# lasgroup/Model-based-policy-optimizers

Measured on AMD Instinct MI355X. Metric: model-rollout transitions/sec + SAC updates/sec, Pendulum 5-ens h=5, higher is better.
Workload: dtype f32

## Files before the change

### include/mbpo_hip.h

```cpp
#ifndef MBPO_HIP_H
#define MBPO_HIP_H

#include <stdint.h>

#ifdef __cplusplus
extern "C" {
#endif

#define MBPO_OK 0
#define MBPO_ERR_ARG (-1)
#define MBPO_ERR_UNSUPPORTED (-2)
#define MBPO_ERR_LAUNCH (-3)

#define MBPO_MAX_LAYERS 8

#define MBPO_ACT_SWISH 0
#define MBPO_ACT_RELU 1
#define MBPO_ACT_TANH 2

typedef struct mbpo_mlp_desc {
  const float *params;
  int64_t net_stride;
  int32_t n_nets;
  int32_t n_layers;
// ... 77 lines not shown
  int32_t ppo_extras, env_major;
  int32_t step_index, n_steps;
  const float *action;
  const float *raw_action;
  const float *log_prob;
  const float *reward;
  const float *x_next;
  const float *sys_done;
  const float *first_obs;
  float *obs, *steps, *done;
  float *transitions;
  int32_t row_len;
} mbpo_episode_step_desc;

int mbpo_episode_step(const mbpo_episode_step_desc *d, void *stream);

int mbpo_replay_insert(float *data, int64_t max_size, int32_t row_len, int32_t *state, const float *rows,
                       int64_t n_rows, void *stream);
int mbpo_replay_gather(const float *data, int64_t max_size, int32_t row_len, const int32_t *state, const int32_t *idx,
                       int64_t n, float *out, void *stream);
int mbpo_replay_sample(const float *data, int64_t max_size, int32_t row_len, const int32_t *state, uint64_t seed,
                       uint64_t offset, const uint64_t *rng_dev, int64_t n, int32_t *idx_out, float *out, void *stream);

int mbpo_philox_permutation(uint64_t seed, uint64_t offset, const uint64_t *rng_dev, int64_t n, int32_t *perm,
                            uint32_t *workspace, void *stream);

int64_t mbpo_running_stats_workspace_floats(int32_t x_dim);
int mbpo_running_stats_reduce(const float *rows, int64_t n_rows, int32_t row_len, int32_t col_off, int32_t x_dim,
                              const float *stats, float *sums, float *workspace, int32_t pass, void *stream);
int mbpo_running_stats_apply(float *stats, const float *sums, int32_t x_dim, float std_min, float std_max, void *stream);
int mbpo_running_stats_update(const float *rows, int64_t n_rows, int32_t row_len, int32_t col_off, int32_t x_dim, float *stats,
                              float *sums, float *workspace, float std_min, float std_max, void *stream);

int mbpo_gae_scan(const float *truncation, const float *termination, const float *rewards, const float *values,
                  const float *bootstrap, float *vs, float *advantages, int64_t B, int32_t T, float gamma,
                  float lam, int32_t time_major, void *stream);
int mbpo_lambda_return_scan(const float *rewards, const float *next_values, float *returns, int64_t B, int32_t T,
                            float gamma, float lam, int32_t time_major, void *stream);
int mbpo_gae_scan_discounts(const float *truncation, const float *termination, const float *rewards, const float *values,
                            const float *bootstrap, const float *discounts, float *vs, float *advantages, int64_t B,
                            int32_t T, float lam, int32_t time_major, void *stream);

typedef struct mbpo_sac_desc {
  int32_t x_dim, u_dim;
  int32_t policy_layers;
  int32_t policy_dims[MBPO_MAX_LAYERS + 1];
  int32_t q_layers;
  int32_t q_dims[MBPO_MAX_LAYERS + 1];
  int32_t policy_activation, q_activation;
  float *params, *target_q, *adam_m, *adam_v, *step_count, *grads;
  float *workspace;
  float *metrics;
  float *metrics_accum;
  const float *batch;
  int32_t batch_size, row_len;
  const float *norm_mean, *norm_std;
  const float *noise_alpha, *noise_critic, *noise_actor;
  uint64_t seed, offset;
  const uint64_t *rng_dev;
  float discounting, reward_scaling, target_entropy, tau;
  float lr_policy, lr_q, lr_alpha, wd_policy, wd_q, wd_alpha, max_grad_norm;
  float grad_scale;
  int32_t non_equidistant_time;
  float continuous_discounting, min_time_between_switches, max_time_between_switches, env_dt;
} mbpo_sac_desc;

// ... 157 lines not shown
```

### model-based-policy-optimizers_amd/csrc/replay.hip

```cpp
#include "common.hpp"
#include <stdlib.h>

struct ReplayPos {
  int pos, roll, head;
};

__device__ __forceinline__ ReplayPos replay_plan(const int *state, long long max_size, long long n) {
  ReplayPos p;
  long long pos = state[0];
  long long roll = max_size - pos - n;
  if (roll > 0) roll = 0;
  p.roll = (int)roll;
  p.pos = (int)(pos + roll);
  p.head = (int)(((long long)state[2] - roll) % max_size);
  return p;
}

__global__ void __launch_bounds__(256) k_replay_insert(float *data, long long max_size, int D, const int *state,
                                                        const float *rows, long long n_rows) {
  const ReplayPos p = replay_plan(state, max_size, n_rows);
  const long long s0 = ((long long)p.pos + p.head) % max_size;
  const long long n1 = (max_size - s0) < n_rows ? (max_size - s0) : n_rows;
  const long long e1 = n1 * D, total = n_rows * D;
  float *dst1 = data + s0 * D;
  const long long gtid = (long long)blockIdx.x * blockDim.x + threadIdx.x, gsz = (long long)gridDim.x * blockDim.x;
  const bool vec = ((e1 | total) & 3) == 0 && ((((unsigned long long)dst1) | ((unsigned long long)data) | ((unsigned long long)rows)) & 15ull) == 0;
  if (vec) {
    const f32x4 *src = reinterpret_cast<const f32x4 *>(rows);
    f32x4 *d1 = reinterpret_cast<f32x4 *>(dst1), *d2 = reinterpret_cast<f32x4 *>(data);
    const long long q1 = e1 >> 2, qt = total >> 2;
    for (long long i = gtid; i < qt; i += gsz) {
      const f32x4 v = src[i];
      if (i < q1) d1[i] = v;
      else d2[i - q1] = v;
    }
  } else {
    for (long long i = gtid; i < total; i += gsz) {
      const float v = rows[i];
      if (i < e1) dst1[i] = v;
      else data[i - e1] = v;
    }
  }
}

__global__ void k_replay_advance(int *state, long long max_size, long long n_rows) {
  if (threadIdx.x == 0 && blockIdx.x == 0) {
    const ReplayPos p = replay_plan(state, max_size, n_rows);
    long long newpos = ((long long)p.pos + n_rows) % (max_size + 1);
    long long sp = (long long)state[1] + p.roll;
    state[0] = (int)newpos;
    state[1] = (int)(sp > 0 ? sp : 0);
    state[2] = p.head;
    state[3] = (int)((unsigned)state[3] + (unsigned)n_rows);
  }
}

extern "C" int mbpo_replay_insert(float *data, int64_t max_size, int32_t row_len, int32_t *state, const float *rows,
                                  int64_t n_rows, void *stream) {
  MBPO_REQUIRE(data && state, MBPO_ERR_ARG, "replay_insert: null pointer");
  MBPO_REQUIRE(max_size > 0 && max_size < (1LL << 31) - 1 && row_len > 0, MBPO_ERR_ARG, "replay_insert: bad max_size/row_len");
  MBPO_REQUIRE(n_rows >= 0 && n_rows <= max_size, MBPO_ERR_ARG,
               "replay_insert: %lld rows do not fit a buffer of %lld rows", (long long)n_rows, (long long)max_size);
  if (n_rows == 0) return MBPO_OK;
  MBPO_REQUIRE(rows, MBPO_ERR_ARG, "replay_insert: null rows");
  long long total = n_rows * row_len;
  int grid = (int)((total + 255) / 256 < 2048 ? (total + 255) / 256 : 2048);
  hipStream_t st = (hipStream_t)stream;
  hipLaunchKernelGGL(k_replay_insert, dim3(grid), dim3(256), 0, st, data, (long long)max_size, row_len, state, rows,
                     (long long)n_rows);
  hipLaunchKernelGGL(k_replay_advance, dim3(1), dim3(64), 0, st, state, (long long)max_size, (long long)n_rows);
  MBPO_CHECK_LAUNCH("replay_insert");
  return MBPO_OK;
}

static int gather_rows_per_block(int row_len) {
  const int pieces = (row_len & 3) == 0 ? row_len >> 2 : row_len;
  int rb = (2048 + pieces - 1) / pieces;
  return rb < 1 ? 1 : (rb > 256 ? 256 : rb);
}

template <bool SAMPLE>
__global__ void __launch_bounds__(256) k_replay_gather(const float *data, long long max_size, int D, const int *state,
                                                        const int *idx, unsigned long long seed, unsigned long long offset,
                                                        const unsigned long long *rng_dev, long long n, int *idx_out, float *out, int RB) {
  __shared__ long long s_phys[256];
  if (SAMPLE) {
    const RngKey rk = rng_resolve(seed, offset, rng_dev);
    seed = rk.seed;
    offset = rk.offset;
  }
  const int head = state[2];
  const int lo = state[1], hi = state[0];
  const int tid = threadIdx.x;
  const bool vec = (D & 3) == 0 && ((((unsigned long long)data) | ((unsigned long long)out)) & 15ull) == 0;
  for (long long row0 = (long long)blockIdx.x * RB; row0 < n; row0 += (long long)gridDim.x * RB) {
    const long long j = row0 + tid;
    if (tid < RB && j < n) {
      long long li;
      if (SAMPLE) {
        li = philox_randint(seed, offset, MBPO_STREAM_REPLAY, (unsigned long long)j, lo, hi);
        if (idx_out) idx_out[j] = (int)li;
      } else {
        li = idx[j];
      }
      long long w = li % max_size;
      if (w < 0) w += max_size;
      s_phys[tid] = (w + head) % max_size;
    }
    __syncthreads();
    const int rows_here = (int)((n - row0) < RB ? (n - row0) : RB);
    if (vec) {
      const int D4 = D >> 2, total = rows_here * D4;
      const f32x4 *src = reinterpret_cast<const f32x4 *>(data);
      f32x4 *dst = reinterpret_cast<f32x4 *>(out) + row0 * D4;
      for (int e = tid; e < total; e += 256) {
        const int r = e / D4, c = e - r * D4;
        dst[e] = src[s_phys[r] * D4 + c];
      }
    } else {
      const int total = rows_here * D;
      float *dst = out + row0 * D;
      for (int e = tid; e < total; e += 256) {
        const int r = e / D, c = e - r * D;
        dst[e] = data[s_phys[r] * D + c];
      }
    }
    __syncthreads();
  }
}

extern "C" int mbpo_replay_gather(const float *data, int64_t max_size, int32_t row_len, const int32_t *state,
                                  const int32_t *idx, int64_t n, float *out, void *stream) {
  MBPO_REQUIRE(data && state, MBPO_ERR_ARG, "replay_gather: null pointer");
  MBPO_REQUIRE(max_size > 0 && row_len > 0 && n >= 0, MBPO_ERR_ARG, "replay_gather: bad sizes");
  if (n == 0) return MBPO_OK;
  MBPO_REQUIRE(idx && out, MBPO_ERR_ARG, "replay_gather: null idx/out");
  const int RB = gather_rows_per_block(row_len);
  int grid = (int)((n + RB - 1) / RB < 4096 ? (n + RB - 1) / RB : 4096);
  hipLaunchKernelGGL(k_replay_gather<false>, dim3(grid), dim3(256), 0, (hipStream_t)stream, data, (long long)max_size, row_len,
                     state, idx, 0ull, 0ull, (const unsigned long long *)nullptr, (long long)n, (int *)nullptr, out, RB);
  MBPO_CHECK_LAUNCH("replay_gather");
  return MBPO_OK;
}

extern "C" int mbpo_replay_sample(const float *data, int64_t max_size, int32_t row_len, const int32_t *state, uint64_t seed,
                                  uint64_t offset, const uint64_t *rng_dev, int64_t n, int32_t *idx_out, float *out,
                                  void *stream) {
  MBPO_REQUIRE(data && state, MBPO_ERR_ARG, "replay_sample: null pointer");
  MBPO_REQUIRE(max_size > 0 && row_len > 0 && n >= 0, MBPO_ERR_ARG, "replay_sample: bad sizes");
  if (n == 0) return MBPO_OK;
  MBPO_REQUIRE(out, MBPO_ERR_ARG, "replay_sample: null out");
  const int RB = gather_rows_per_block(row_len);
  int grid = (int)((n + RB - 1) / RB < 4096 ? (n + RB - 1) / RB : 4096);
  hipLaunchKernelGGL(k_replay_gather<true>, dim3(grid), dim3(256), 0, (hipStream_t)stream, data, (long long)max_size, row_len,
                     state, (const int *)nullptr, (unsigned long long)seed, (unsigned long long)offset, (const unsigned long long *)rng_dev, (long long)n, idx_out, out, RB);
  MBPO_CHECK_LAUNCH("replay_sample");
  return MBPO_OK;
}

#define STATS_WGS 512

__device__ __forceinline__ float wave_sum(float v) {
#pragma unroll
  for (int o = 32; o > 0; o >>= 1) v += __shfl_down(v, o, 64);
  return v;
}

template <int PASS>
__global__ void __launch_bounds__(256) k_stats_partial(const float *rows, long long n_rows, int D, int col_off, int X,
                                                        const float *stats, const float *sums, float *partial) {
  const int tid = threadIdx.x;
  const float *mean = stats + 1;
  const int rows_per_pass = 256 / X;
  const int c = tid % X, r0 = tid / X;
  float acc = 0.f;
  if (r0 < rows_per_pass) {
    const float m = mean[c];
    float upd = 0.f;
    if (PASS == 1) upd = sums[1 + c] / (stats[0] + sums[0]);
    for (long long r = (long long)blockIdx.x * rows_per_pass + r0; r < n_rows; r += (long long)gridDim.x * rows_per_pass) {
      float d = rows[r * D + col_off + c] - m;
      acc += (PASS == 0) ? d : d * (d - upd);
    }
  }
  __shared__ float s_all[256];
  s_all[tid] = acc;
  __syncthreads();
  if (tid < X) {
    float a = 0.f;
    for (int t = tid; t < rows_per_pass * X; t += X) a += s_all[t];
    partial[(long long)blockIdx.x * X + tid] = a;
  }
}

__device__ __forceinline__ float stats_column_sums(const float *partial, int n_parts, int X, float *s_sl) {
  const int tid = threadIdx.x;
  const int nsl = 256 / X, c = tid % X, sl = tid / X;
  float acc = 0.f;
  if (sl < nsl) {
    int g = sl;
    for (; g + 7 * nsl < n_parts; g += 8 * nsl) {
      float v[8];
#pragma unroll
      for (int k = 0; k < 8; ++k) v[k] = partial[(long long)(g + k * nsl) * X + c];
#pragma unroll
      for (int k = 0; k < 8; ++k) acc += v[k];
    }
    for (; g < n_parts; g += nsl) acc += partial[(long long)g * X + c];
  }
  s_sl[tid] = acc;
  __syncthreads();
  float a = 0.f;
  if (tid < X)
    for (int k = 0; k < nsl; ++k) a += s_sl[k * X + tid];
  __syncthreads();
  return a;
}

template <int PASS>
__global__ void __launch_bounds__(256) k_stats_sums(const float *partial, int n_parts, int X, long long n_rows, float *sums) {
  __shared__ float s_sl[256];
  const int tid = threadIdx.x;
  const float a = stats_column_sums(partial, n_parts, X, s_sl);
  if (tid < X) sums[1 + PASS * X + tid] = a;
  if (PASS == 0 && tid == 0) sums[0] = (float)n_rows;
// ... 21 lines not shown
    hipLaunchKernelGGL(k_stats_sums<0>, dim3(1), dim3(256), 0, st, workspace, grid, x_dim, (long long)n_rows, sums);
  } else {
    hipLaunchKernelGGL(k_stats_partial<1>, dim3(grid), dim3(256), 0, st, rows, (long long)n_rows, row_len, col_off, x_dim, stats,
                       (const float *)sums, workspace);
    hipLaunchKernelGGL(k_stats_sums<1>, dim3(1), dim3(256), 0, st, workspace, grid, x_dim, (long long)n_rows, sums);
  }
  MBPO_CHECK_LAUNCH("running_stats_reduce");
  return MBPO_OK;
}

__global__ void k_stats_apply(float *stats, const float *sums, int X, float std_min, float std_max) {
  const int c = threadIdx.x;
  const float count = stats[0] + sums[0];
  if (c < X && count > 0.f) {
    float *mean = stats + 1, *sv = stats + 1 + X, *sd = stats + 1 + 2 * X;
    mean[c] = mean[c] + sums[1 + c] / count;
    float nsv = sv[c] + sums[1 + X + c];
    sv[c] = nsv;
    float s = sqrtf(fmaxf(nsv, 0.f) / count);
    sd[c] = fminf(fmaxf(s, std_min), std_max);
  }
  __syncthreads();
  if (c == 0) stats[0] = count;
}

extern "C" int mbpo_running_stats_apply(float *stats, const float *sums, int32_t x_dim, float std_min, float std_max, void *stream) {
  MBPO_REQUIRE(stats && sums, MBPO_ERR_ARG, "running_stats_apply: null pointer");
  MBPO_REQUIRE(x_dim > 0 && x_dim <= 128, MBPO_ERR_ARG, "running_stats_apply: x_dim out of range");
  hipLaunchKernelGGL(k_stats_apply, dim3(1), dim3(128), 0, (hipStream_t)stream, stats, sums, x_dim, std_min, std_max);
  MBPO_CHECK_LAUNCH("running_stats_apply");
  return MBPO_OK;
}

__global__ void __launch_bounds__(256) k_stats_pass1_fused(const float *rows, long long n_rows, int D, int col_off, int X,
                                                           const float *stats, const float *partial0, int n_parts0, float *sums,
                                                           float *partial1) {
  __shared__ float s_all[256];
  __shared__ float s_sum0[128];
  const int tid = threadIdx.x;
  const float tot = stats_column_sums(partial0, n_parts0, X, s_all);
  if (tid < X) {
    s_sum0[tid] = tot;
    if (blockIdx.x == 0) sums[1 + tid] = tot;
  }
  if (blockIdx.x == 0 && tid == 0) sums[0] = (float)n_rows;
  __syncthreads();
  const float *mean = stats + 1;
  const int rows_per_pass = 256 / X;
  const int c = tid % X, r0 = tid / X;
  float acc = 0.f;
  if (r0 < rows_per_pass) {
    const float m = mean[c];
    const float upd = s_sum0[c] / (stats[0] + (float)n_rows);
    for (long long r = (long long)blockIdx.x * rows_per_pass + r0; r < n_rows; r += (long long)gridDim.x * rows_per_pass) {
      float d = rows[r * D + col_off + c] - m;
      acc += d * (d - upd);
    }
  }
  s_all[tid] = acc;
  __syncthreads();
  if (tid < X) {
    float a = 0.f;
    for (int t = tid; t < rows_per_pass * X; t += X) a += s_all[t];
    partial1[(long long)blockIdx.x * X + tid] = a;
  }
}

__global__ void __launch_bounds__(256) k_stats_sums1_apply(const float *partial1, int n_parts, int X, float *sums, float *stats,
                                                           float std_min, float std_max) {
  __shared__ float s_sl[256];
  const int c = threadIdx.x;
  const float a = stats_column_sums(partial1, n_parts, X, s_sl);
  const float count = stats[0] + sums[0];
  if (c < X) {
    sums[1 + X + c] = a;
    if (count > 0.f) {
      float *mean = stats + 1, *sv = stats + 1 + X, *sd = stats + 1 + 2 * X;
      mean[c] = mean[c] + sums[1 + c] / count;
      float nsv = sv[c] + a;
      sv[c] = nsv;
      float s = sqrtf(fmaxf(nsv, 0.f) / count);
      sd[c] = fminf(fmaxf(s, std_min), std_max);
    }
  }
  __syncthreads();
  if (c == 0) stats[0] = count;
}

extern "C" int mbpo_running_stats_update(const float *rows, int64_t n_rows, int32_t row_len, int32_t col_off, int32_t x_dim,
                                         float *stats, float *sums, float *workspace, float std_min, float std_max, void *stream) {
  MBPO_REQUIRE(stats && sums && workspace, MBPO_ERR_ARG, "running_stats_update: null pointer");
  MBPO_REQUIRE(x_dim > 0 && x_dim <= 128 && row_len > 0 && col_off >= 0 && col_off + x_dim <= row_len, MBPO_ERR_ARG,
               "running_stats_update: bad column range (x_dim must be <= 128)");
  MBPO_REQUIRE(n_rows >= 0 && (n_rows == 0 || rows), MBPO_ERR_ARG, "running_stats_update: bad rows");
  hipStream_t st = (hipStream_t)stream;
  int rows_per_pass = 256 / x_dim;
  long long want = (n_rows + rows_per_pass - 1) / rows_per_pass;
  int grid = (int)(want < 1 ? 1 : (want < STATS_WGS ? want : STATS_WGS));
  float *partial1 = workspace + (long long)STATS_WGS * x_dim;
  hipLaunchKernelGGL(k_stats_partial<0>, dim3(grid), dim3(256), 0, st, rows, (long long)n_rows, row_len, col_off, x_dim,
                     (const float *)stats, (const float *)sums, workspace);
  hipLaunchKernelGGL(k_stats_pass1_fused, dim3(grid), dim3(256), 0, st, rows, (long long)n_rows, row_len, col_off, x_dim,
                     (const float *)stats, (const float *)workspace, grid, sums, partial1);
  hipLaunchKernelGGL(k_stats_sums1_apply, dim3(1), dim3(256), 0, st, (const float *)partial1, grid, x_dim, sums, stats, std_min, std_max);
  MBPO_CHECK_LAUNCH("running_stats_update");
  return MBPO_OK;
}

__global__ void __launch_bounds__(256) k_perm_keys(unsigned long long seed, unsigned long long offset, const unsigned long long *rng_dev,
                                                    long long n, unsigned int *keys) {
  const RngKey rk = rng_resolve(seed, offset, rng_dev);
  const long long i = (long long)blockIdx.x * 256 + threadIdx.x;
  if (i >= n) return;
  Philox4 p = philox4x32_10((uint32_t)i, (uint32_t)((unsigned long long)i >> 32), MBPO_STREAM_PERM ^ (uint32_t)(rk.offset >> 32) * 0x9E3779B9u,
                            (uint32_t)rk.offset, (uint32_t)rk.seed, (uint32_t)(rk.seed >> 32));
  keys[i] = p.v[0];
}

__global__ void __launch_bounds__(256) k_perm_rank(const unsigned int *keys, long long n, int *perm) {
  __shared__ unsigned int s_k[1024];
  const long long i = (long long)blockIdx.x * 256 + threadIdx.x;
  const unsigned int ki = i < n ? keys[i] : 0u;
  int rank = 0;
  for (long long j0 = 0; j0 < n; j0 += 1024) {
    __syncthreads();
    for (int t = threadIdx.x; t < 1024; t += 256) s_k[t] = (j0 + t < n) ? keys[j0 + t] : 0xFFFFFFFFu;
    __syncthreads();
    const int m = (int)((n - j0) < 1024 ? (n - j0) : 1024);
    for (int t = 0; t < m; ++t) {
      const unsigned int kj = s_k[t];
      rank += (kj < ki || (kj == ki && j0 + t < i)) ? 1 : 0;
    }
  }
  if (i < n) perm[rank] = (int)i;
}

__global__ void __launch_bounds__(1024) k_perm_sort_lds(unsigned long long seed, unsigned long long offset, const unsigned long long *rng_dev,
                                                         int n, int np, int *perm, unsigned int *flag) {
// ... 123 lines not shown
```

### model-based-policy-optimizers_amd/mbpo/_hip.py

```python
from __future__ import annotations

import ctypes as C
import os
from pathlib import Path
from typing import Optional, Sequence

import torch

MBPO_MAX_LAYERS = 8
ACT_IDS = {"swish": 0, "silu": 0, "relu": 1, "tanh": 2}

SYS_PENDULUM, SYS_ENSEMBLE = 0, 1
SYS_GENERIC = 100
ENS_MEAN, ENS_TS1, ENS_TSINF = 0, 1, 2
STREAM_POLICY_NOISE, STREAM_MODEL_NOISE, STREAM_MEMBER = 1, 2, 3
REWARD_PENDULUM, REWARD_QUADRATIC, REWARD_LEARNED = 0, 1, 2

_LIB_PATH = Path(__file__).resolve().parent / "_lib" / "libmbpo_hip.so"


class P2pDesc(C.Structure):
    _fields_ = [("world", C.c_int32), ("rank", C.c_int32), ("n_max", C.c_int64), ("regions", C.c_void_p * 16)]


# ... 138 lines not shown


def load() -> C.CDLL:
    global _lib
    if _lib is not None:
        return _lib
    p = lib_path()
    if not p.exists():
        raise MbpoHipError(
            f"{p} not found: build it with `python model-based-policy-optimizers_amd/build.py` "
            "(needs hipcc; this framework has no CPU fallback)")
    lib = C.CDLL(str(p))
    lib.mbpo_version.restype = C.c_int
    lib.mbpo_last_error.restype = C.c_char_p
    lib.mbpo_ensemble_mlp_forward.restype = C.c_int
    lib.mbpo_ensemble_mlp_forward.argtypes = [C.POINTER(MlpDesc), C.c_void_p, C.c_int32, C.c_void_p, C.c_int64,
                                              C.c_void_p]
    lib.mbpo_model_rollout.restype = C.c_int
    lib.mbpo_model_rollout.argtypes = [C.POINTER(RolloutDesc), C.c_void_p]
    _bind_optional(lib)
    _lib = lib
    return lib


def _bind_optional(lib: C.CDLL) -> None:
    i32, i64, u64, f32, vp = C.c_int32, C.c_int64, C.c_uint64, C.c_float, C.c_void_p
    sigs = {
        "mbpo_replay_insert": [vp, i64, i32, vp, vp, i64, vp],
        "mbpo_replay_gather": [vp, i64, i32, vp, vp, i64, vp, vp],
        "mbpo_replay_sample": [vp, i64, i32, vp, u64, u64, vp, i64, vp, vp, vp],
        "mbpo_running_stats_reduce": [vp, i64, i32, i32, i32, vp, vp, vp, i32, vp],
        "mbpo_running_stats_apply": [vp, vp, i32, f32, f32, vp],
        "mbpo_running_stats_update": [vp, i64, i32, i32, i32, vp, vp, vp, f32, f32, vp],
        "mbpo_gae_scan": [vp, vp, vp, vp, vp, vp, vp, i64, i32, f32, f32, i32, vp],
        "mbpo_gae_scan_discounts": [vp, vp, vp, vp, vp, vp, vp, vp, i64, i32, f32, i32, vp],
        "mbpo_lambda_return_scan": [vp, vp, vp, i64, i32, f32, f32, i32, vp],
        "mbpo_critic_grads": [vp, i32, i32, vp, i32, vp, i32, vp, vp, i64, vp, vp, vp, vp, vp, vp],
        "mbpo_adamw_step": [vp, vp, vp, vp, vp, i64, f32, f32, f32, i32, vp, f32, vp, vp, vp],
        "mbpo_rng_advance": [vp, u64, vp],
        "mbpo_soft_update": [vp, vp, vp, i64, f32, vp],
        "mbpo_philox_permutation": [u64, u64, vp, i64, vp, vp, vp],
    }
    for name, argtypes in sigs.items():
        fn = getattr(lib, name, None)
        if fn is not None:
            fn.restype = C.c_int
            fn.argtypes = argtypes
    for name in ("mbpo_sac_grads", "mbpo_sac_grad_norms", "mbpo_sac_apply", "mbpo_sac_step", "mbpo_sac_finalize"):
        fn = getattr(lib, name, None)
        if fn is not None:
            fn.restype = C.c_int
            fn.argtypes = [C.POINTER(SacDesc), vp]
    fn = getattr(lib, "mbpo_sac_finalize_advance", None)
    if fn is not None:
        fn.restype = C.c_int
        fn.argtypes = [C.POINTER(SacDesc), vp, u64, vp]
    for name in ("mbpo_ppo_grads", "mbpo_ppo_apply", "mbpo_ppo_step"):
        fn = getattr(lib, name, None)
        if fn is not None:
            fn.restype = C.c_int
            fn.argtypes = [C.POINTER(PpoDesc), vp]
    fn = getattr(lib, "mbpo_ppo_workspace_floats", None)
    if fn is not None:
        fn.restype = C.c_int64
        fn.argtypes = [C.POINTER(PpoDesc)]
    fn = getattr(lib, "mbpo_critic_workspace_floats", None)
# ... 122 lines not shown
```

### model-based-policy-optimizers_amd/mbpo/ops.py

```python
from __future__ import annotations

import ctypes as C
import os
from dataclasses import dataclass
from typing import Optional, Sequence

import torch

from . import _hip
from ._hip import check, current_stream_ptr, load, mlp_desc, ptr, require_device_tensor as _req


@dataclass
class MlpSpec:
    dims: Sequence[int]
    activation: str = "swish"
    n_nets: int = 1

    @property
    def n_params(self) -> int:
        d = list(self.dims)
        return sum(d[i] * d[i + 1] + d[i + 1] for i in range(len(d) - 1))

    @property
# ... 467 lines not shown
                         std_min: float = 1e-6, std_max: float = 1e6) -> None:
    if all_reduce is None:
        lib = load()
        _req(rows, "rows"); _req(stats, "stats")
        if rows.dim() != 2 or stats.numel() != 1 + 3 * x_dim:
            raise ValueError("rows must be [n, row_len] and stats [1 + 3*x_dim]")
        if sums is None:
            sums = torch.zeros(1 + 2 * x_dim, device=rows.device, dtype=torch.float32)
        if workspace is None:
            workspace = torch.empty(stats_workspace_floats(x_dim), device=rows.device, dtype=torch.float32)
        _req(sums, "sums"); _req(workspace, "workspace")
        if workspace.numel() < stats_workspace_floats(x_dim):
            raise ValueError(f"workspace must hold {stats_workspace_floats(x_dim)} floats, got {workspace.numel()}")
        check(lib.mbpo_running_stats_update(rows.data_ptr(), rows.shape[0], rows.shape[1], col_off, x_dim, stats.data_ptr(),
                                            sums.data_ptr(), workspace.data_ptr(), std_min, std_max, current_stream_ptr()),
              "mbpo_running_stats_update")
        return
    sums = running_stats_reduce(rows, col_off, x_dim, stats, 0, sums=sums, workspace=workspace)
    if all_reduce is not None:
        all_reduce(sums)
    running_stats_reduce(rows, col_off, x_dim, stats, 1, sums=sums, workspace=workspace)
    if all_reduce is not None:
        all_reduce(sums[1 + x_dim:])
    running_stats_apply(stats, sums, x_dim, std_min, std_max)


def running_stats_apply(stats: torch.Tensor, sums: torch.Tensor, x_dim: int, std_min: float = 1e-6, std_max: float = 1e6) -> None:
    lib = load()
    _req(stats, "stats"); _req(sums, "sums")
    check(lib.mbpo_running_stats_apply(stats.data_ptr(), sums.data_ptr(), x_dim, std_min, std_max, current_stream_ptr()),
          "mbpo_running_stats_apply")


def gae_scan(truncation, termination, rewards, values, bootstrap, gamma, lam: float, time_major: bool = False):
    lib = load()
    for t, nm in ((truncation, "truncation"), (termination, "termination"), (rewards, "rewards"), (values, "values"),
                  (bootstrap, "bootstrap")):
        _req(t, nm)
    B, T = (values.shape[1], values.shape[0]) if time_major else (values.shape[0], values.shape[1])
    if bootstrap.shape != (B,):
        raise ValueError("bootstrap must be [B]")
    vs = torch.empty_like(values)
    adv = torch.empty_like(values)
    if isinstance(gamma, torch.Tensor):
        _req(gamma, "gamma")
        if gamma.shape != values.shape:
            raise ValueError("a per-element discount must have the shape of rewards/values")
        check(lib.mbpo_gae_scan_discounts(truncation.data_ptr(), termination.data_ptr(), rewards.data_ptr(), values.data_ptr(),
                                          bootstrap.data_ptr(), gamma.data_ptr(), vs.data_ptr(), adv.data_ptr(), B, T, lam,
                                          int(time_major), current_stream_ptr()), "mbpo_gae_scan_discounts")
        return vs, adv
    check(lib.mbpo_gae_scan(truncation.data_ptr(), termination.data_ptr(), rewards.data_ptr(), values.data_ptr(),
                            bootstrap.data_ptr(), vs.data_ptr(), adv.data_ptr(), B, T, gamma, lam, int(time_major),
                            current_stream_ptr()), "mbpo_gae_scan")
    return vs, adv


def lambda_return_scan(rewards, next_values, gamma: float, lam: float, time_major: bool = False):
    lib = load()
    _req(rewards, "rewards"); _req(next_values, "next_values")
    B, T = (rewards.shape[1], rewards.shape[0]) if time_major else (rewards.shape[0], rewards.shape[1])
    out = torch.empty_like(rewards)
    check(lib.mbpo_lambda_return_scan(rewards.data_ptr(), next_values.data_ptr(), out.data_ptr(), B, T, gamma, lam,
                                      int(time_major), current_stream_ptr()), "mbpo_lambda_return_scan")
    return out

# ... 573 lines not shown
```

### model-based-policy-optimizers_amd/mbpo/optimizers/policy_optimizers/sac/sac.py

```python
from __future__ import annotations

import dataclasses
import math
import os
import time
from dataclasses import dataclass
from typing import Any, Callable, Dict, List, Optional, Sequence, Tuple

import torch

from mbpo import _hip, ops
from mbpo.optimizers.policy_optimizers.brax_utils.base import State
from mbpo.parallel import DataParallel
from mbpo.replay import ReplayBufferState, UniformSamplingQueue
from mbpo.systems.brax_wrapper import BraxWrapper
from mbpo.systems.ensemble_system import lecun_uniform_flat
from mbpo.types import Transition
from mbpo.utils import keys as K

Metrics = Dict[str, Any]

SITE_ROLLOUT, SITE_SAMPLE, SITE_SGD = 1, 2, 16


# ... 195 lines not shown

        return policy

    def _norm(self, normalizer_params: RunningStatisticsState):
        if not self.normalize_observations:
            return None, None
        return normalizer_params.mean.contiguous(), normalizer_params.std.contiguous()

    def init_training_state(self, key: int) -> TrainingState:
        key_policy, key_q = K.split(key)
        gp = torch.Generator().manual_seed(key_policy % (2 ** 63))
        gq = torch.Generator().manual_seed(key_q % (2 ** 63))
        pol = ops.embed_mlp_params(lecun_uniform_flat(self.policy_dims_logical, gp), self.policy_dims_logical, self.kernel_width)
        q = torch.cat([ops.embed_mlp_params(lecun_uniform_flat(self.q_dims_logical, gq), self.q_dims_logical, self.q_width)
                       for _ in range(2)])
        params = torch.cat([pol, q, torch.tensor([self.init_log_alpha], dtype=torch.float32)]).to(self.device)
        self.dp.broadcast(params, src=0)
        self.updater.load_state(params)
        self._stats_vec.zero_()
        self._stats_vec[1 + 2 * self.x_dim:] = 1.0
        return self._training_state(env_steps=0)

    def _training_state(self, env_steps: int) -> TrainingState:
        u = self.updater
        return TrainingState(policy_optimizer_state=(u.adam_m[:u.P], u.adam_v[:u.P]), policy_params=u.policy_params,
                             q_optimizer_state=(u.adam_m[u.P:u.P + 2 * u.Q], u.adam_v[u.P:u.P + 2 * u.Q]),
                             q_params=u.q_params, target_q_params=u.target_q, gradient_steps=u.step_count,
                             env_steps=env_steps, alpha_optimizer_state=(u.adam_m[-1:], u.adam_v[-1:]),
                             alpha_params=u.log_alpha, normalizer_params=RunningStatisticsState(self._stats_vec, self.x_dim))

    def rekey(self, key: int) -> None:
        ops.set_rng(self._rng, K.PRNGKey(key), 0)

    def get_experience(self, normalizer_params: RunningStatisticsState, policy_params: torch.Tensor, env_state: State,
                       buffer_state: ReplayBufferState, key: Optional[int] = None):
        if key is not None:
            self.rekey(key)
        nm, ns = self._norm(normalizer_params)
        spec = self.env.system.rollout_spec(env_state.system_params, self.device)
        sp_out: list = []
        rows = ops.model_rollout(policy_params=policy_params, policy_spec=self.policy_spec, x_dim=self.x_dim, u_dim=self.u_dim,
                                 obs=env_state.obs, first_obs=env_state.info['first_obs'], steps=env_state.info['steps'],
                                 done=env_state.done, n_steps=self.num_env_steps_between_updates,
                                 episode_length=self.episode_length, action_repeat=self.action_repeat, norm_mean=nm,
                                 norm_std=ns, seed=0, offset=SITE_ROLLOUT << 32, rng_dev=self._rng,
                                 out=self._rollout_rows, system_params_out=sp_out, **spec)
        if sp_out:
            env_state = env_state.replace(system_params=sp_out[-1])
        ops.running_stats_update(rows, 0, self.x_dim, normalizer_params.vec, all_reduce=self._all_reduce,
                                 sums=self._stats_sums, workspace=self._stats_ws)
        buffer_state = self.replay_buffer.insert_rows(buffer_state, rows)
        return normalizer_params, env_state, buffer_state

    def sgd_step(self, transitions_rows: torch.Tensor, normalizer_params: RunningStatisticsState, key: Optional[int] = None,
                 g: int = 0, defer_clip_check: bool = False) -> None:
        if key is not None:
            self.rekey(key)
        nm, ns = self._norm(normalizer_params)
        self.updater.sgd_step(transitions_rows, nm, ns, seed=0, offset=(SITE_SGD + g) << 32, rng_dev=self._rng,
                              defer_clip_check=defer_clip_check)

    def training_step(self, training_state: TrainingState, env_state: State, buffer_state: ReplayBufferState,
                      key: Optional[int] = None):
        if key is not None:
            self.rekey(key)
        normalizer_params, env_state, buffer_state = self.get_experience(
            training_state.normalizer_params, training_state.policy_params, env_state, buffer_state)
        training_state = training_state.replace(
            env_steps=training_state.env_steps + self.env_steps_per_actor_step * self.num_env_steps_between_updates)
        buffer_state, rows = self.replay_buffer.sample_rows(buffer_state, out=self._batch_rows, seed=0,
                                                            offset=SITE_SAMPLE << 32, rng_dev=self._rng)
        B = self.batch_size
        for g in range(self.grad_updates_per_step):
            self.sgd_step(rows[g * B:(g + 1) * B], normalizer_params, g=g, defer_clip_check=True)
        self.updater.finalize(rng_dev=self._rng)
        return training_state, env_state, buffer_state

    def prefill_replay_buffer(self, training_state: TrainingState, env_state: State, buffer_state: ReplayBufferState, key: int):
        key, new_key = K.split(key)
        self.rekey(key)
        for _ in range(self.num_prefill_actor_steps):
            _, env_state, buffer_state = self.get_experience(training_state.normalizer_params, training_state.policy_params,
                                                             env_state, buffer_state)
            ops.rng_advance(self._rng)
            training_state = training_state.replace(env_steps=training_state.env_steps + self.env_steps_per_actor_step)
        return training_state, env_state, buffer_state, new_key

    def training_epoch(self, training_state: TrainingState, env_state: State, buffer_state: ReplayBufferState, key: int):
        self.updater.metrics_accum.zero_()
        n = self.num_training_steps_per_epoch
        env_steps_per = self.env_steps_per_actor_step * self.num_env_steps_between_updates
        done_steps = 0
        self.rekey(key)
        if self.use_graph and self._capturable():
            gkey, refs = self._graph_signature(training_state, env_state, buffer_state)
            if self._graph is None or self._graph_key != gkey:
                training_state, env_state, buffer_state = self.training_step(training_state, env_state, buffer_state)
                done_steps = 1
                gkey, refs = self._graph_signature(training_state, env_state, buffer_state)
                torch.cuda.synchronize()
                graph = torch.cuda.CUDAGraph()
                with torch.cuda.graph(graph):
                    self.training_step(training_state, env_state, buffer_state)
                self._graph, self._graph_key, self._graph_refs = graph, gkey, refs
# ... 171 lines not shown
```

### model-based-policy-optimizers_amd/mbpo/replay.py

```python
from __future__ import annotations

import dataclasses
from dataclasses import dataclass
from typing import Optional, Tuple

import torch

from . import ops
from .types import Transition, flatten, row_layout, unflatten
from .utils import keys as K


@dataclass
class ReplayBufferState:
    data: torch.Tensor
    state: torch.Tensor
    key: int
    insert_position: int = 0
    sample_position: int = 0
    head: int = 0
    sample_count: int = 0

    def replace(self, **kw):
        return dataclasses.replace(self, **kw)
# ... 14 lines not shown
            d.observation.device if d.observation.is_cuda else torch.device("cuda", torch.cuda.current_device()))

    def init(self, key: int) -> ReplayBufferState:
        data = torch.zeros(self.max_replay_size, self.row_len, device=self.device, dtype=torch.float32)
        state = torch.zeros(4, device=self.device, dtype=torch.int32)
        return ReplayBufferState(data=data, state=state, key=K.PRNGKey(key))

    def insert(self, buffer_state: ReplayBufferState, samples) -> ReplayBufferState:
        rows = samples if isinstance(samples, torch.Tensor) else flatten(samples)
        return self.insert_rows(buffer_state, rows)

    def sample(self, buffer_state: ReplayBufferState) -> Tuple[ReplayBufferState, Transition]:
        st, rows = self.sample_rows(buffer_state)
        return st, unflatten(rows, self.x_dim, self.u_dim, self.has_truncation, self.ppo_extras)

    def size(self, buffer_state: ReplayBufferState) -> int:
        return buffer_state.insert_position - buffer_state.sample_position

    def insert_rows(self, bs: ReplayBufferState, rows: torch.Tensor) -> ReplayBufferState:
        n = rows.shape[0]
        if n > self.max_replay_size:
            raise ValueError(f"cannot insert {n} rows into a buffer of {self.max_replay_size}")
        ops.replay_insert(bs.data, bs.state, rows.to(self.device).contiguous())
        return self.insert_mirror(bs, n)

    def insert_mirror(self, bs: ReplayBufferState, n: int) -> ReplayBufferState:
        mx = self.max_replay_size
        roll = min(0, mx - bs.insert_position - n)
        pos = bs.insert_position + roll
        return bs.replace(insert_position=(pos + n) % (mx + 1), sample_position=max(0, bs.sample_position + roll),
                          head=(bs.head - roll) % mx)

    def sample_rows(self, bs: ReplayBufferState, n: Optional[int] = None, out: Optional[torch.Tensor] = None,
                    rng_dev: Optional[torch.Tensor] = None, seed: Optional[int] = None, offset: int = 0
                    ) -> Tuple[ReplayBufferState, torch.Tensor]:
        n = self.sample_batch_size if n is None else n
        if self.size(bs) <= 0:
            raise ValueError("cannot sample from an empty replay buffer")
        key, sample_key = K.split(bs.key)
        rows = ops.replay_sample(bs.data, bs.state, n, seed=sample_key if seed is None else seed, offset=offset, out=out,
                                 rng_dev=rng_dev)
        return bs.replace(key=key, sample_count=bs.sample_count + 1), rows

    def logical_data(self, bs: ReplayBufferState) -> torch.Tensor:
        idx = (torch.arange(self.max_replay_size, device=bs.data.device) + bs.head) % self.max_replay_size
        return bs.data[idx]
```

Baseline: 18.82 million.

## Fuse replay insert/advance and sampling into the running-stats kernels

```diff
diff --git a/include/mbpo_hip.h b/include/mbpo_hip.h
--- a/include/mbpo_hip.h
+++ b/include/mbpo_hip.h
@@ -133,6 +133,13 @@
 int mbpo_running_stats_update(const float *rows, int64_t n_rows, int32_t row_len, int32_t col_off, int32_t x_dim, float *stats,
                               float *sums, float *workspace, float std_min, float std_max, void *stream);
 
+int mbpo_stats_insert(const float *rows, int64_t n_rows, int32_t row_len, int32_t col_off, int32_t x_dim, float *stats, float *sums,
+                      float *workspace, float std_min, float std_max, float *data, int64_t max_size, int32_t *state,
+                      int32_t defer_apply, void *stream);
+int mbpo_sample_stats_apply(const float *data, int64_t max_size, int32_t row_len, const int32_t *state, uint64_t seed, uint64_t offset,
+                            const uint64_t *rng_dev, int64_t n, int32_t *idx_out, float *out, int64_t n_rows_stats, int32_t x_dim,
+                            float *stats, float *sums, const float *workspace, float std_min, float std_max, void *stream);
+
 int mbpo_gae_scan(const float *truncation, const float *termination, const float *rewards, const float *values,
                   const float *bootstrap, float *vs, float *advantages, int64_t B, int32_t T, float gamma,
                   float lam, int32_t time_major, void *stream);
diff --git a/model-based-policy-optimizers_amd/csrc/replay.hip b/model-based-policy-optimizers_amd/csrc/replay.hip
--- a/model-based-policy-optimizers_amd/csrc/replay.hip
+++ b/model-based-policy-optimizers_amd/csrc/replay.hip
@@ -16,8 +16,8 @@
   return p;
 }
 
-__global__ void __launch_bounds__(256) k_replay_insert(float *data, long long max_size, int D, const int *state,
-                                                        const float *rows, long long n_rows) {
+__device__ __forceinline__ void replay_insert_copy(float *data, long long max_size, int D, const int *state, const float *rows,
+                                                   long long n_rows) {
   const ReplayPos p = replay_plan(state, max_size, n_rows);
   const long long s0 = ((long long)p.pos + p.head) % max_size;
   const long long n1 = (max_size - s0) < n_rows ? (max_size - s0) : n_rows;
@@ -43,16 +43,23 @@
   }
 }
 
+__global__ void __launch_bounds__(256) k_replay_insert(float *data, long long max_size, int D, const int *state,
+                                                        const float *rows, long long n_rows) {
+  replay_insert_copy(data, max_size, D, state, rows, n_rows);
+}
+
+__device__ __forceinline__ void replay_advance_state(int *state, long long max_size, long long n_rows) {
+  const ReplayPos p = replay_plan(state, max_size, n_rows);
+  long long newpos = ((long long)p.pos + n_rows) % (max_size + 1);
+  long long sp = (long long)state[1] + p.roll;
+  state[0] = (int)newpos;
+  state[1] = (int)(sp > 0 ? sp : 0);
+  state[2] = p.head;
+  state[3] = (int)((unsigned)state[3] + (unsigned)n_rows);
+}
+
 __global__ void k_replay_advance(int *state, long long max_size, long long n_rows) {
-  if (threadIdx.x == 0 && blockIdx.x == 0) {
-    const ReplayPos p = replay_plan(state, max_size, n_rows);
-    long long newpos = ((long long)p.pos + n_rows) % (max_size + 1);
-    long long sp = (long long)state[1] + p.roll;
-    state[0] = (int)newpos;
-    state[1] = (int)(sp > 0 ? sp : 0);
-    state[2] = p.head;
-    state[3] = (int)((unsigned)state[3] + (unsigned)n_rows);
-  }
+  if (threadIdx.x == 0 && blockIdx.x == 0) replay_advance_state(state, max_size, n_rows);
 }
 
 extern "C" int mbpo_replay_insert(float *data, int64_t max_size, int32_t row_len, int32_t *state, const float *rows,
@@ -80,10 +87,9 @@
 }
 
 template <bool SAMPLE>
-__global__ void __launch_bounds__(256) k_replay_gather(const float *data, long long max_size, int D, const int *state,
-                                                        const int *idx, unsigned long long seed, unsigned long long offset,
-                                                        const unsigned long long *rng_dev, long long n, int *idx_out, float *out, int RB) {
-  __shared__ long long s_phys[256];
+__device__ __forceinline__ void replay_gather_rows(const float *data, long long max_size, int D, const int *state, const int *idx,
+                                                   unsigned long long seed, unsigned long long offset, const unsigned long long *rng_dev,
+                                                   long long n, int *idx_out, float *out, int RB, long long *s_phys, int bid, int nblk) {
   if (SAMPLE) {
     const RngKey rk = rng_resolve(seed, offset, rng_dev);
     seed = rk.seed;
@@ -93,7 +99,7 @@
   const int lo = state[1], hi = state[0];
   const int tid = threadIdx.x;
   const bool vec = (D & 3) == 0 && ((((unsigned long long)data) | ((unsigned long long)out)) & 15ull) == 0;
-  for (long long row0 = (long long)blockIdx.x * RB; row0 < n; row0 += (long long)gridDim.x * RB) {
+  for (long long row0 = (long long)bid * RB; row0 < n; row0 += (long long)nblk * RB) {
     const long long j = row0 + tid;
     if (tid < RB && j < n) {
       long long li;
@@ -129,6 +135,15 @@
   }
 }
 
+template <bool SAMPLE>
+__global__ void __launch_bounds__(256) k_replay_gather(const float *data, long long max_size, int D, const int *state,
+                                                        const int *idx, unsigned long long seed, unsigned long long offset,
+                                                        const unsigned long long *rng_dev, long long n, int *idx_out, float *out, int RB) {
+  __shared__ long long s_phys[256];
+  replay_gather_rows<SAMPLE>(data, max_size, D, state, idx, seed, offset, rng_dev, n, idx_out, out, RB, s_phys, (int)blockIdx.x,
+                             (int)gridDim.x);
+}
+
 extern "C" int mbpo_replay_gather(const float *data, int64_t max_size, int32_t row_len, const int32_t *state,
                                   const int32_t *idx, int64_t n, float *out, void *stream) {
   MBPO_REQUIRE(data && state, MBPO_ERR_ARG, "replay_gather: null pointer");
@@ -167,8 +182,8 @@
 }
 
 template <int PASS>
-__global__ void __launch_bounds__(256) k_stats_partial(const float *rows, long long n_rows, int D, int col_off, int X,
-                                                        const float *stats, const float *sums, float *partial) {
+__device__ __forceinline__ void stats_partial_wg(const float *rows, long long n_rows, int D, int col_off, int X, const float *stats,
+                                                 const float *sums, float *partial, float *s_all) {
   const int tid = threadIdx.x;
   const float *mean = stats + 1;
   const int rows_per_pass = 256 / X;
@@ -183,7 +198,6 @@
       acc += (PASS == 0) ? d : d * (d - upd);
     }
   }
-  __shared__ float s_all[256];
   s_all[tid] = acc;
   __syncthreads();
   if (tid < X) {
@@ -191,6 +205,13 @@
     for (int t = tid; t < rows_per_pass * X; t += X) a += s_all[t];
     partial[(long long)blockIdx.x * X + tid] = a;
   }
+}
+
+template <int PASS>
+__global__ void __launch_bounds__(256) k_stats_partial(const float *rows, long long n_rows, int D, int col_off, int X,
+                                                        const float *stats, const float *sums, float *partial) {
+  __shared__ float s_all[256];
+  stats_partial_wg<PASS>(rows, n_rows, D, col_off, X, stats, sums, partial, s_all);
 }
 
 __device__ __forceinline__ float stats_column_sums(const float *partial, int n_parts, int X, float *s_sl) {
@@ -278,11 +299,9 @@
   return MBPO_OK;
 }
 
-__global__ void __launch_bounds__(256) k_stats_pass1_fused(const float *rows, long long n_rows, int D, int col_off, int X,
-                                                           const float *stats, const float *partial0, int n_parts0, float *sums,
-                                                           float *partial1) {
-  __shared__ float s_all[256];
-  __shared__ float s_sum0[128];
+__device__ __forceinline__ void stats_pass1_fused_wg(const float *rows, long long n_rows, int D, int col_off, int X, const float *stats,
+                                                     const float *partial0, int n_parts0, float *sums, float *partial1, float *s_all,
+                                                     float *s_sum0) {
   const int tid = threadIdx.x;
   const float tot = stats_column_sums(partial0, n_parts0, X, s_all);
   if (tid < X) {
@@ -312,9 +331,16 @@
   }
 }
 
-__global__ void __launch_bounds__(256) k_stats_sums1_apply(const float *partial1, int n_parts, int X, float *sums, float *stats,
-                                                           float std_min, float std_max) {
-  __shared__ float s_sl[256];
+__global__ void __launch_bounds__(256) k_stats_pass1_fused(const float *rows, long long n_rows, int D, int col_off, int X,
+                                                           const float *stats, const float *partial0, int n_parts0, float *sums,
+                                                           float *partial1) {
+  __shared__ float s_all[256];
+  __shared__ float s_sum0[128];
+  stats_pass1_fused_wg(rows, n_rows, D, col_off, X, stats, partial0, n_parts0, sums, partial1, s_all, s_sum0);
+}
+
+__device__ __forceinline__ void stats_sums1_apply_wg(const float *partial1, int n_parts, int X, float *sums, float *stats, float std_min,
+                                                     float std_max, float *s_sl) {
   const int c = threadIdx.x;
   const float a = stats_column_sums(partial1, n_parts, X, s_sl);
   const float count = stats[0] + sums[0];
@@ -331,6 +357,12 @@
   }
   __syncthreads();
   if (c == 0) stats[0] = count;
+}
+
+__global__ void __launch_bounds__(256) k_stats_sums1_apply(const float *partial1, int n_parts, int X, float *sums, float *stats,
+                                                           float std_min, float std_max) {
+  __shared__ float s_sl[256];
+  stats_sums1_apply_wg(partial1, n_parts, X, sums, stats, std_min, std_max, s_sl);
 }
 
 extern "C" int mbpo_running_stats_update(const float *rows, int64_t n_rows, int32_t row_len, int32_t col_off, int32_t x_dim,
@@ -350,6 +382,111 @@
                      (const float *)stats, (const float *)workspace, grid, sums, partial1);
   hipLaunchKernelGGL(k_stats_sums1_apply, dim3(1), dim3(256), 0, st, (const float *)partial1, grid, x_dim, sums, stats, std_min, std_max);
   MBPO_CHECK_LAUNCH("running_stats_update");
+  return MBPO_OK;
+}
+
+static int g_step_frontend = -1;
+extern "C" int mbpo_debug_set_step_frontend(int mode) {
+  MBPO_REQUIRE(mode >= -1 && mode <= 1, MBPO_ERR_ARG, "debug_set_step_frontend: mode must be -1 (default), 0 (separate launches) or 1 (paired)");
+  g_step_frontend = mode;
+  return MBPO_OK;
+}
+
+__global__ void __launch_bounds__(256) k_stats_pass0_insert(const float *rows, long long n_rows, int D, int col_off, int X,
+                                                            const float *stats, float *partial0, float *data, long long max_size,
+                                                            const int *state) {
+  __shared__ float s_all[256];
+  replay_insert_copy(data, max_size, D, state, rows, n_rows);
+  stats_partial_wg<0>(rows, n_rows, D, col_off, X, stats, (const float *)nullptr, partial0, s_all);
+}
+
+__global__ void __launch_bounds__(256) k_stats_pass1_advance(const float *rows, long long n_rows, int D, int col_off, int X,
+                                                             const float *stats, const float *partial0, int n_parts0, float *sums,
+                                                             float *partial1, int *state, long long max_size) {
+  __shared__ float s_all[256];
+  __shared__ float s_sum0[128];
+  if (blockIdx.x == gridDim.x - 1 && threadIdx.x == 0) replay_advance_state(state, max_size, n_rows);
+  stats_pass1_fused_wg(rows, n_rows, D, col_off, X, stats, partial0, n_parts0, sums, partial1, s_all, s_sum0);
+}
+
+__global__ void __launch_bounds__(256) k_sample_stats_apply(const float *data, long long max_size, int D, const int *state,
+                                                            unsigned long long seed, unsigned long long offset,
+                                                            const unsigned long long *rng_dev, long long n, int *idx_out, float *out, int RB,
+                                                            const float *partial1, int n_parts, int X, float *sums, float *stats,
+                                                            float std_min, float std_max) {
+  __shared__ long long s_phys[256];
+  __shared__ float s_sl[256];
+  if (blockIdx.x == 0) {
+    stats_sums1_apply_wg(partial1, n_parts, X, sums, stats, std_min, std_max, s_sl);
+    return;
+  }
+  replay_gather_rows<true>(data, max_size, D, state, (const int *)nullptr, seed, offset, rng_dev, n, idx_out, out, RB, s_phys,
+                           (int)blockIdx.x - 1, (int)gridDim.x - 1);
+}
+
+static int stats_grid(int64_t n_rows, int32_t x_dim) {
+  int rows_per_pass = 256 / x_dim;
+  long long want = (n_rows + rows_per_pass - 1) / rows_per_pass;
+  return (int)(want < 1 ? 1 : (want < STATS_WGS ? want : STATS_WGS));
+}
+
+extern "C" int mbpo_stats_insert(const float *rows, int64_t n_rows, int32_t row_len, int32_t col_off, int32_t x_dim, float *stats,
+                                 float *sums, float *workspace, float std_min, float std_max, float *data, int64_t max_size,
+                                 int32_t *state, int32_t defer_apply, void *stream) {
+  MBPO_REQUIRE(stats && sums && workspace && data && state && rows, MBPO_ERR_ARG, "stats_insert: null pointer");
+  MBPO_REQUIRE(x_dim > 0 && x_dim <= 128 && row_len > 0 && col_off >= 0 && col_off + x_dim <= row_len, MBPO_ERR_ARG,
+               "stats_insert: bad column range (x_dim must be <= 128)");
+  MBPO_REQUIRE(max_size > 0 && max_size < (1LL << 31) - 1, MBPO_ERR_ARG, "stats_insert: bad max_size");
+  MBPO_REQUIRE(n_rows > 0 && n_rows <= max_size, MBPO_ERR_ARG, "stats_insert: %lld rows do not fit a buffer of %lld rows",
+               (long long)n_rows, (long long)max_size);
+  hipStream_t st = (hipStream_t)stream;
+  if (g_step_frontend == 0) {
+    if (defer_apply) {
+      const int grid = stats_grid(n_rows, x_dim);
+      hipLaunchKernelGGL(k_stats_partial<0>, dim3(grid), dim3(256), 0, st, rows, (long long)n_rows, row_len, col_off, x_dim,
+                         (const float *)stats, (const float *)sums, workspace);
+      hipLaunchKernelGGL(k_stats_pass1_fused, dim3(grid), dim3(256), 0, st, rows, (long long)n_rows, row_len, col_off, x_dim,
+                         (const float *)stats, (const float *)workspace, grid, sums, workspace + (long long)STATS_WGS * x_dim);
+      MBPO_CHECK_LAUNCH("stats_insert");
+    } else {
+      int rc = mbpo_running_stats_update(rows, n_rows, row_len, col_off, x_dim, stats, sums, workspace, std_min, std_max, stream);
+      if (rc != MBPO_OK) return rc;
+    }
+    return mbpo_replay_insert(data, max_size, row_len, state, rows, n_rows, stream);
+  }
+  const int grid = stats_grid(n_rows, x_dim);
+  float *partial1 = workspace + (long long)STATS_WGS * x_dim;
+  hipLaunchKernelGGL(k_stats_pass0_insert, dim3(grid), dim3(256), 0, st, rows, (long long)n_rows, row_len, col_off, x_dim,
+                     (const float *)stats, workspace, data, (long long)max_size, (const int *)state);
+  hipLaunchKernelGGL(k_stats_pass1_advance, dim3(grid), dim3(256), 0, st, rows, (long long)n_rows, row_len, col_off, x_dim,
+                     (const float *)stats, (const float *)workspace, grid, sums, partial1, state, (long long)max_size);
+  if (!defer_apply)
+    hipLaunchKernelGGL(k_stats_sums1_apply, dim3(1), dim3(256), 0, st, (const float *)partial1, grid, x_dim, sums, stats, std_min, std_max);
+  MBPO_CHECK_LAUNCH("stats_insert");
+  return MBPO_OK;
+}
+
+extern "C" int mbpo_sample_stats_apply(const float *data, int64_t max_size, int32_t row_len, const int32_t *state, uint64_t seed,
+                                       uint64_t offset, const uint64_t *rng_dev, int64_t n, int32_t *idx_out, float *out,
+                                       int64_t n_rows_stats, int32_t x_dim, float *stats, float *sums, const float *workspace,
+                                       float std_min, float std_max, void *stream) {
+  MBPO_REQUIRE(data && state && out && stats && sums && workspace, MBPO_ERR_ARG, "sample_stats_apply: null pointer");
+  MBPO_REQUIRE(max_size > 0 && row_len > 0 && n > 0, MBPO_ERR_ARG, "sample_stats_apply: bad sizes");
+  MBPO_REQUIRE(x_dim > 0 && x_dim <= 128 && n_rows_stats > 0, MBPO_ERR_ARG, "sample_stats_apply: bad x_dim / n_rows_stats");
+  hipStream_t st = (hipStream_t)stream;
+  const int n_parts = stats_grid(n_rows_stats, x_dim);
+  const float *partial1 = workspace + (long long)STATS_WGS * x_dim;
+  if (g_step_frontend == 0) {
+    hipLaunchKernelGGL(k_stats_sums1_apply, dim3(1), dim3(256), 0, st, partial1, n_parts, x_dim, sums, stats, std_min, std_max);
+    MBPO_CHECK_LAUNCH("sample_stats_apply");
+    return mbpo_replay_sample(data, max_size, row_len, state, seed, offset, rng_dev, n, idx_out, out, stream);
+  }
+  const int RB = gather_rows_per_block(row_len);
+  int grid = (int)((n + RB - 1) / RB < 4096 ? (n + RB - 1) / RB : 4096);
+  hipLaunchKernelGGL(k_sample_stats_apply, dim3(grid + 1), dim3(256), 0, st, data, (long long)max_size, row_len, (const int *)state,
+                     (unsigned long long)seed, (unsigned long long)offset, (const unsigned long long *)rng_dev, (long long)n, idx_out, out,
+                     RB, partial1, n_parts, x_dim, sums, stats, std_min, std_max);
+  MBPO_CHECK_LAUNCH("sample_stats_apply");
   return MBPO_OK;
 }
 
diff --git a/model-based-policy-optimizers_amd/mbpo/_hip.py b/model-based-policy-optimizers_amd/mbpo/_hip.py
--- a/model-based-policy-optimizers_amd/mbpo/_hip.py
+++ b/model-based-policy-optimizers_amd/mbpo/_hip.py
@@ -194,6 +194,8 @@
         "mbpo_running_stats_reduce": [vp, i64, i32, i32, i32, vp, vp, vp, i32, vp],
         "mbpo_running_stats_apply": [vp, vp, i32, f32, f32, vp],
         "mbpo_running_stats_update": [vp, i64, i32, i32, i32, vp, vp, vp, f32, f32, vp],
+        "mbpo_stats_insert": [vp, i64, i32, i32, i32, vp, vp, vp, f32, f32, vp, i64, vp, i32, vp],
+        "mbpo_sample_stats_apply": [vp, i64, i32, vp, u64, u64, vp, i64, vp, vp, i64, i32, vp, vp, vp, f32, f32, vp],
         "mbpo_gae_scan": [vp, vp, vp, vp, vp, vp, vp, i64, i32, f32, f32, i32, vp],
         "mbpo_gae_scan_discounts": [vp, vp, vp, vp, vp, vp, vp, vp, i64, i32, f32, i32, vp],
         "mbpo_lambda_return_scan": [vp, vp, vp, i64, i32, f32, f32, i32, vp],
diff --git a/model-based-policy-optimizers_amd/mbpo/ops.py b/model-based-policy-optimizers_amd/mbpo/ops.py
--- a/model-based-policy-optimizers_amd/mbpo/ops.py
+++ b/model-based-policy-optimizers_amd/mbpo/ops.py
@@ -523,6 +523,38 @@
           "mbpo_running_stats_apply")
 
 
+def stats_insert(rows: torch.Tensor, col_off: int, x_dim: int, stats: torch.Tensor, sums: torch.Tensor, workspace: torch.Tensor,
+                 data: torch.Tensor, state: torch.Tensor, defer_apply: bool = False, std_min: float = 1e-6,
+                 std_max: float = 1e6) -> None:
+    lib = load()
+    _req(rows, "rows"); _req(stats, "stats"); _req(sums, "sums"); _req(workspace, "workspace")
+    _req(data, "data"); _req(state, "state", torch.int32)
+    if rows.dim() != 2 or rows.shape[1] != data.shape[1] or stats.numel() != 1 + 3 * x_dim or sums.numel() < 1 + 2 * x_dim:
+        raise ValueError(f"rows must be [n,{data.shape[1]}], stats [1 + 3*x_dim] and sums [1 + 2*x_dim]")
+    if workspace.numel() < stats_workspace_floats(x_dim):
+        raise ValueError(f"workspace must hold {stats_workspace_floats(x_dim)} floats, got {workspace.numel()}")
+    check(lib.mbpo_stats_insert(rows.data_ptr(), rows.shape[0], rows.shape[1], col_off, x_dim, stats.data_ptr(), sums.data_ptr(),
+                                workspace.data_ptr(), std_min, std_max, data.data_ptr(), data.shape[0], state.data_ptr(),
+                                int(bool(defer_apply)), current_stream_ptr()), "mbpo_stats_insert")
+
+
+def replay_sample_stats_apply(data: torch.Tensor, state: torch.Tensor, n: int, seed: int, offset: int, out: torch.Tensor,
+                              rng_dev: Optional[torch.Tensor], n_rows_stats: int, x_dim: int, stats: torch.Tensor,
+                              sums: torch.Tensor, workspace: torch.Tensor, std_min: float = 1e-6,
+                              std_max: float = 1e6) -> torch.Tensor:
+    lib = load()
+    _req(data, "data"); _req(state, "state", torch.int32); _req(out, "out")
+    _req(stats, "stats"); _req(sums, "sums"); _req(workspace, "workspace")
+    if out.numel() != n * data.shape[1] or stats.numel() != 1 + 3 * x_dim or sums.numel() < 1 + 2 * x_dim:
+        raise ValueError(f"out must hold {n} rows of {data.shape[1]} floats, stats [1 + 3*x_dim] and sums [1 + 2*x_dim]")
+    if workspace.numel() < stats_workspace_floats(x_dim):
+        raise ValueError(f"workspace must hold {stats_workspace_floats(x_dim)} floats, got {workspace.numel()}")
+    check(lib.mbpo_sample_stats_apply(data.data_ptr(), data.shape[0], data.shape[1], state.data_ptr(), seed, offset, rng_ptr(rng_dev),
+                                      n, None, out.data_ptr(), n_rows_stats, x_dim, stats.data_ptr(), sums.data_ptr(),
+                                      workspace.data_ptr(), std_min, std_max, current_stream_ptr()), "mbpo_sample_stats_apply")
+    return out
+
+
 def gae_scan(truncation, termination, rewards, values, bootstrap, gamma, lam: float, time_major: bool = False):
     lib = load()
     for t, nm in ((truncation, "truncation"), (termination, "termination"), (rewards, "rewards"), (values, "values"),
diff --git a/model-based-policy-optimizers_amd/mbpo/optimizers/policy_optimizers/sac/sac.py b/model-based-policy-optimizers_amd/mbpo/optimizers/policy_optimizers/sac/sac.py
--- a/model-based-policy-optimizers_amd/mbpo/optimizers/policy_optimizers/sac/sac.py
+++ b/model-based-policy-optimizers_amd/mbpo/optimizers/policy_optimizers/sac/sac.py
@@ -251,8 +251,11 @@
     def rekey(self, key: int) -> None:
         ops.set_rng(self._rng, K.PRNGKey(key), 0)
 
+    def _paired_front_end(self) -> bool:
+        return self._all_reduce is None and 0 < self._rollout_rows.shape[0] <= self.replay_buffer.max_replay_size
+
     def get_experience(self, normalizer_params: RunningStatisticsState, policy_params: torch.Tensor, env_state: State,
-                       buffer_state: ReplayBufferState, key: Optional[int] = None):
+                       buffer_state: ReplayBufferState, key: Optional[int] = None, defer_stats_apply: bool = False):
         if key is not None:
             self.rekey(key)
         nm, ns = self._norm(normalizer_params)
@@ -266,6 +269,10 @@
                                  out=self._rollout_rows, system_params_out=sp_out, **spec)
         if sp_out:
             env_state = env_state.replace(system_params=sp_out[-1])
+        if self._paired_front_end():
+            ops.stats_insert(rows, 0, self.x_dim, normalizer_params.vec, self._stats_sums, self._stats_ws, buffer_state.data,
+                             buffer_state.state, defer_apply=defer_stats_apply)
+            return normalizer_params, env_state, self.replay_buffer.insert_mirror(buffer_state, rows.shape[0])
         ops.running_stats_update(rows, 0, self.x_dim, normalizer_params.vec, all_reduce=self._all_reduce,
                                  sums=self._stats_sums, workspace=self._stats_ws)
         buffer_state = self.replay_buffer.insert_rows(buffer_state, rows)
@@ -283,12 +290,16 @@
                       key: Optional[int] = None):
         if key is not None:
             self.rekey(key)
+        paired = self._paired_front_end()
         normalizer_params, env_state, buffer_state = self.get_experience(
-            training_state.normalizer_params, training_state.policy_params, env_state, buffer_state)
+            training_state.normalizer_params, training_state.policy_params, env_state, buffer_state, defer_stats_apply=paired)
         training_state = training_state.replace(
             env_steps=training_state.env_steps + self.env_steps_per_actor_step * self.num_env_steps_between_updates)
+        pending = dict(n_rows_stats=self._rollout_rows.shape[0], x_dim=self.x_dim, stats=normalizer_params.vec,
+                       sums=self._stats_sums, workspace=self._stats_ws) if paired else None
         buffer_state, rows = self.replay_buffer.sample_rows(buffer_state, out=self._batch_rows, seed=0,
-                                                            offset=SITE_SAMPLE << 32, rng_dev=self._rng)
+                                                            offset=SITE_SAMPLE << 32, rng_dev=self._rng,
+                                                            pending_stats=pending)
         B = self.batch_size
         for g in range(self.grad_updates_per_step):
             self.sgd_step(rows[g * B:(g + 1) * B], normalizer_params, g=g, defer_clip_check=True)
diff --git a/model-based-policy-optimizers_amd/mbpo/replay.py b/model-based-policy-optimizers_amd/mbpo/replay.py
--- a/model-based-policy-optimizers_amd/mbpo/replay.py
+++ b/model-based-policy-optimizers_amd/mbpo/replay.py
@@ -70,14 +70,20 @@
                           head=(bs.head - roll) % mx)
 
     def sample_rows(self, bs: ReplayBufferState, n: Optional[int] = None, out: Optional[torch.Tensor] = None,
-                    rng_dev: Optional[torch.Tensor] = None, seed: Optional[int] = None, offset: int = 0
-                    ) -> Tuple[ReplayBufferState, torch.Tensor]:
+                    rng_dev: Optional[torch.Tensor] = None, seed: Optional[int] = None, offset: int = 0,
+                    pending_stats: Optional[dict] = None) -> Tuple[ReplayBufferState, torch.Tensor]:
         n = self.sample_batch_size if n is None else n
         if self.size(bs) <= 0:
             raise ValueError("cannot sample from an empty replay buffer")
         key, sample_key = K.split(bs.key)
-        rows = ops.replay_sample(bs.data, bs.state, n, seed=sample_key if seed is None else seed, offset=offset, out=out,
-                                 rng_dev=rng_dev)
+        if pending_stats is not None:
+            if out is None:
+                out = torch.empty((n, self.row_len), device=bs.data.device, dtype=torch.float32)
+            rows = ops.replay_sample_stats_apply(bs.data, bs.state, n, seed=sample_key if seed is None else seed, offset=offset,
+                                                 out=out, rng_dev=rng_dev, **pending_stats)
+        else:
+            rows = ops.replay_sample(bs.data, bs.state, n, seed=sample_key if seed is None else seed, offset=offset, out=out,
+                                     rng_dev=rng_dev)
         return bs.replace(key=key, sample_count=bs.sample_count + 1), rows
 
     def logical_data(self, bs: ReplayBufferState) -> torch.Tensor:
```

After: 18.54 million. -1.5%, worse.
